# cloneofsimo/paint-with-words-sd

Measured on NVIDIA H100. Metric: unet_steps_per_sec_512sq_cfg, higher is better.
Workload: dtype f16

## Files before the change

paint_with_words_sd_b200/csrc/pww_abi.cu:

```cuda
#include <stdio.h>
#include <string.h>

#include "pww_common.cuh"
#include "xattn_tc.cuh"
#include "xattn_fused2.cuh"
#include "attn_tc.cuh"
#include "unet_ops.cuh"
#include "sampler_step.cuh"
#include "control_inject.cuh"
#include "control_combine.cuh"
#include <stdlib.h>
#include <algorithm>
#include <type_traits>

namespace {

thread_local char g_last_cuda_error[640] = "";

int cuda_fail(cudaError_t e);

bool aligned16(const void* p) { return (reinterpret_cast<uintptr_t>(p) & 15u) == 0; }

bool supported_head_dim(int D) { return D == 40 || D == 64 || D == 80 || D == 160; }

int check_common(const void* q, const void* k, int B, int H, int N, int T, int D, int64_t q_bs, int64_t q_rs,
                 int64_t k_bs, int64_t k_rs) {
  if (!q || !k || B <= 0 || H <= 0 || N <= 0 || T <= 0 || D <= 0) return PWW_ERR_BAD_ARG;
  if (!aligned16(q) || !aligned16(k)) return PWW_ERR_BAD_ARG;
  if ((q_bs | q_rs | k_bs | k_rs) & 7) return PWW_ERR_BAD_ARG;
  if (q_rs < (int64_t)H * D || k_rs < (int64_t)H * D) return PWW_ERR_BAD_ARG;
  if (!supported_head_dim(D) || !pww::core::supported_keys(T)) return PWW_ERR_UNSUPPORTED;
  return PWW_OK;
}

template <int D_, int KC_>
struct Shape {
  static constexpr int D = D_, KC = KC_;
};
template <int D, typename F>
cudaError_t with_chunks(int T, F&& f) {
  switch (pww::core::chunks_of(T)) {
    case 1: return f(Shape<D, 1>{});
    case 2: return f(Shape<D, 2>{});
    case 3: return f(Shape<D, 3>{});
  }
  return cudaErrorInvalidValue;
}
template <typename F>
cudaError_t with_shape(int D, int T, F&& f) {
  switch (D) {
    case 40: return with_chunks<40>(T, f);
    case 64: return with_chunks<64>(T, f);
    case 80: return with_chunks<80>(T, f);
    case 160: return with_chunks<160>(T, f);
  }
  return cudaErrorInvalidValue;
}

template <int lo, int hi, typename F>
void with_int(int v, F&& f) {
  if constexpr (lo < hi)
    if (v != lo) return with_int<lo + 1, hi>(v, f);
  f(std::integral_constant<int, lo>{});
}

size_t align_up(size_t x, size_t a) { return (x + a - 1) / a * a; }

constexpr int kStatSlotsPerImage = 2048;

int cuda_fail(cudaError_t e) {
  snprintf(g_last_cuda_error, sizeof(g_last_cuda_error), "%s: %s ", cudaGetErrorName(e), cudaGetErrorString(e));
  return PWW_ERR_CUDA;
}

template <typename E>
pww::XattnParams<E> xattn_params(const void* q, const void* k, const void* v, void* out, int B, int H, int N, int T, int D,
                                 int64_t q_bs, int64_t q_rs, int64_t k_bs, int64_t k_rs, int64_t o_bs, int64_t o_rs) {
  pww::XattnParams<E> p;
  memset(&p, 0, sizeof(p));
  p.q = (const E*)q; p.k = (const E*)k; p.v = (const E*)v; p.out = (E*)out;
  p.B = B; p.H = H; p.N = N; p.T = T; p.D = D;
  p.q_bs = q_bs; p.q_rs = q_rs; p.k_bs = k_bs; p.k_rs = k_rs; p.o_bs = o_bs; p.o_rs = o_rs;
  return p;
}

template <typename E>
pww::XattnParams<E> images(const pww::XattnParams<E>& p, int b0, int n) {
  pww::XattnParams<E> c = p;
  c.B = n;
  c.q += (int64_t)b0 * p.q_bs;
  c.k += (int64_t)b0 * p.k_bs;
  if (c.v) c.v += (int64_t)b0 * p.k_bs;
  if (c.out) c.out += (int64_t)b0 * p.o_bs;
  if (c.wmap_index) c.wmap_index += b0;
  if (c.stat_kind) c.stat_kind += b0;
  if (c.stats) c.stats += b0;
  if (c.stats_out) c.stats_out += b0;
  if (c.g_sigma) c.g_sigma += (int64_t)b0 * p.g_stride;
  return c;
}

}

extern "C" {

int pww_version(void) { return 300; }

const char* pww_status_str(int status) {
  switch (status) {
    case PWW_OK: return "ok";
    case PWW_ERR_BAD_ARG: return "bad argument (null/misaligned pointer, non-positive size or stride not a multiple of 8)";
    case PWW_ERR_UNSUPPORTED: return "unsupported shape or dtype (head dim must be 40/64/80/160, T <= 80, 154 or 231)";
    case PWW_ERR_CUDA: return "CUDA error (see pww_last_cuda_error)";
    case PWW_ERR_WORKSPACE: return "workspace too small (see pww_xattn_workspace_bytes)";
    default: return "unknown status";
  }
}

const char* pww_last_cuda_error(void) { return g_last_cuda_error; }

int pww_device_supported(void) {
  int dev = 0, major = 0;
  cudaError_t e = cudaGetDevice(&dev);
  if (e != cudaSuccess) return cuda_fail(e);
  e = cudaDeviceGetAttribute(&major, cudaDevAttrComputeCapabilityMajor, dev);
  if (e != cudaSuccess) return cuda_fail(e);
  return major == 9 ? 1 : 0;
}

size_t pww_xattn_workspace_bytes(int B, int H, int N, int T, int D) {
  (void)T; (void)D;
  if (B <= 0 || H <= 0 || N <= 0) return 0;
  return align_up((size_t)B * sizeof(unsigned int), 256) +
         (size_t)B * kStatSlotsPerImage * sizeof(pww::StatPartial);
}

}

namespace {

template <typename E>
int xattn_stats(const void* q, const void* k, int B, int H, int N, int T, int D, int64_t q_batch_stride,
                int64_t q_row_stride, int64_t k_batch_stride, int64_t k_row_stride, int stat, const int32_t* kinds,
                bool per_image, const int32_t* wmap_index, float* stats, void* workspace, size_t workspace_bytes,
                void* stream) {
  int rc = check_common(q, k, B, H, N, T, D, q_batch_stride, q_row_stride, k_batch_stride, k_row_stride);
  if (rc) return rc;
  if (!stats || !workspace) return PWW_ERR_BAD_ARG;
  if (per_image ? !kinds : (stat != PWW_STAT_MAX && stat != PWW_STAT_STD)) return PWW_ERR_BAD_ARG;
  if (workspace_bytes < pww_xattn_workspace_bytes(B, H, N, T, D)) return PWW_ERR_WORKSPACE;
  if (pww::num_sms() > kStatSlotsPerImage) return PWW_ERR_WORKSPACE;
  pww::XattnParams<E> p = xattn_params<E>(q, k, nullptr, nullptr, B, H, N, T, D, q_batch_stride, q_row_stride,
                                          k_batch_stride, k_row_stride, 0, 0);
  p.wmap_index = wmap_index; p.stat = stat; p.stat_kind = per_image ? kinds : nullptr; p.stats_out = stats;
  p.counters = (unsigned int*)workspace;
  p.partials = (pww::StatPartial*)((char*)workspace + align_up((size_t)B * sizeof(unsigned int), 256));
  for (int b0 = 0; b0 < B; b0 += pww::tc::kMaxBatch) {
    const pww::XattnParams<E> c = images(p, b0, std::min(B - b0, pww::tc::kMaxBatch));
    const cudaError_t e =
        with_shape(D, T, [&](auto k) { return pww::tc::launch_stats<k.D, k.KC>(c, (cudaStream_t)stream); });
    if (e != cudaSuccess) return cuda_fail(e);
  }
  return PWW_OK;
}

template <typename E>
int xattn_fwd(const void* q, const void* k, const void* v, void* out, int B, int H, int N, int T, int D,
              int64_t q_batch_stride, int64_t q_row_stride, int64_t k_batch_stride, int64_t k_row_stride,
              int64_t o_batch_stride, int64_t o_row_stride, const float* wmap, int64_t wmap_batch_stride,
              const int32_t* wmap_index, const float* stats, const float* g_sigma, int64_t g_stride, float scale,
              void* stream) {
  int rc = check_common(q, k, B, H, N, T, D, q_batch_stride, q_row_stride, k_batch_stride, k_row_stride);
  if (rc) return rc;
  if (!v || !out || !aligned16(v) || !aligned16(out)) return PWW_ERR_BAD_ARG;
  if ((o_batch_stride | o_row_stride) & 7 || o_row_stride < (int64_t)H * D) return PWW_ERR_BAD_ARG;
  if (wmap && (!stats || !g_sigma)) return PWW_ERR_BAD_ARG;
  pww::XattnParams<E> p = xattn_params<E>(q, k, v, out, B, H, N, T, D, q_batch_stride, q_row_stride, k_batch_stride,
                                          k_row_stride, o_batch_stride, o_row_stride);
  p.wmap = wmap; p.wmap_bs = wmap_batch_stride; p.wmap_index = wmap ? wmap_index : nullptr;
  p.stats = stats; p.g_sigma = g_sigma; p.g_stride = g_stride; p.scale = scale;
  for (int b0 = 0; b0 < B; b0 += pww::tc::kMaxBatch) {
    pww::XattnParams<E> c = images(p, b0, std::min(B - b0, pww::tc::kMaxBatch));
    if (wmap && !wmap_index) c.wmap += (int64_t)b0 * wmap_batch_stride;
    const cudaError_t e =
        with_shape(D, T, [&](auto k) { return pww::tc::launch_fwd<k.D, k.KC>(c, (cudaStream_t)stream); });
    if (e != cudaSuccess) return cuda_fail(e);
  }
  return PWW_OK;
}

template <typename E>
int xattn_fused(const void* q, const void* k, const void* v, void* out, int B, int H, int N, int T, int D,
                int64_t q_batch_stride, int64_t q_row_stride, int64_t k_batch_stride, int64_t k_row_stride,
                int64_t o_batch_stride, int64_t o_row_stride, const void* mpack, int64_t mpack_batch_stride, int Bw,
                const int8_t* cidx, const int32_t* wmap_index, int stat, const int32_t* kinds, bool per_image,
                const float* g_sigma, float scale, float* stats, void* workspace, size_t workspace_bytes,
                void* stream) {
  int rc = check_common(q, k, B, H, N, T, D, q_batch_stride, q_row_stride, k_batch_stride, k_row_stride);
  if (rc) return rc;
  if (!v || !out || !aligned16(v) || !aligned16(out)) return PWW_ERR_BAD_ARG;
  if ((o_batch_stride | o_row_stride) & 7 || o_row_stride < (int64_t)H * D || o_batch_stride <= 0) return PWW_ERR_BAD_ARG;
  if (mpack) {
    if (!cidx || !g_sigma || !workspace || Bw <= 0 || !aligned16(mpack)) return PWW_ERR_BAD_ARG;
    if ((mpack_batch_stride & 7) || mpack_batch_stride < (int64_t)N * pww::fx::kMW) return PWW_ERR_BAD_ARG;
    if (per_image ? !kinds : (stat != PWW_STAT_MAX && stat != PWW_STAT_STD)) return PWW_ERR_BAD_ARG;
    if (workspace_bytes < pww_xattn_fused_workspace_bytes()) return PWW_ERR_WORKSPACE;
  }
  pww::XattnParams<E> p = xattn_params<E>(q, k, v, out, B, H, N, T, D, q_batch_stride, q_row_stride, k_batch_stride,
                                          k_row_stride, o_batch_stride, o_row_stride);
  p.g_sigma = g_sigma; p.g_stride = per_image ? 1 : 0; p.scale = scale; p.stat = stat;
  p.stat_kind = per_image ? kinds : nullptr; p.stats_out = stats;
  p.wmap_index = mpack ? wmap_index : nullptr;
  p.counters = (unsigned int*)workspace;
  p.partials = workspace ? (pww::StatPartial*)((char*)workspace + 512) : nullptr;
  int chunk = pww::fx::kMaxBatch;
  const int tiles = pww::ceil_div(N, pww::core::kBM);
  const int hg = pww::ceil_div(H, D == 40 ? pww::fx::Cfg2<40>::G : (D == 64 ? pww::fx::Cfg2<64>::G : 1));
  while (chunk > 1) {
    const int cb = B < chunk ? B : chunk;
    if (pww::fx::fused2_fits(cb, hg, tiles, pww::fx::fused_grid(cb * hg * tiles))) break;
    chunk >>= 1;
  }
  for (int b0 = 0; b0 < B; b0 += chunk) {
    pww::XattnParams<E> c = images(p, b0, std::min(B - b0, chunk));
    const void* mp = mpack;
    const int8_t* ci = cidx;
    if (mpack && !wmap_index) {
      mp = (const __half*)mpack + (int64_t)b0 * mpack_batch_stride;
      ci = cidx + (int64_t)b0 * pww::core::kTP * pww::core::chunks_of(T);
    }
    c.wmap = (const float*)mp;
    const cudaError_t e = with_shape(D, T, [&](auto k) {
      return pww::fx::launch_fused2<k.D, k.KC>(c, mp, mpack_batch_stride, ci, (cudaStream_t)stream);
    });
    if (e == cudaErrorInvalidConfiguration) return PWW_ERR_UNSUPPORTED;
    if (e != cudaSuccess) return cuda_fail(e);
  }
  return PWW_OK;
}

template <typename E>
int groupnorm_nhwc(const void* x, const void* add, int64_t add_batch_stride, const void* gamma, const void* beta, void* y,
                   int B, int HW, int C, int G, float eps, int silu, void* workspace, size_t workspace_bytes,
                   void* stream) {
  if (!x || !gamma || !beta || !y || !workspace || B <= 0 || HW <= 0 || C <= 0 || G <= 0) return PWW_ERR_BAD_ARG;
  if (!aligned16(x) || !aligned16(y) || !aligned16(gamma) || !aligned16(beta) || (add && !aligned16(add)))
    return PWW_ERR_BAD_ARG;
  if ((C & 7) || (C % G) || G > 64 || (C >> 3) > 1024) return PWW_ERR_UNSUPPORTED;
  if (add && ((add_batch_stride & 7) || add_batch_stride < C)) return PWW_ERR_BAD_ARG;
  if (workspace_bytes < pww_groupnorm_workspace_bytes(B, HW, G)) return PWW_ERR_WORKSPACE;
  pww::uops::GnParams<E> p;
  p.x = (const E*)x; p.add = (const E*)add; p.add_bs = add_batch_stride; p.gamma = (const E*)gamma; p.beta = (const E*)beta;
  p.y = (E*)y;
  char* w = (char*)workspace;
  p.counters = (unsigned int*)w;
  w += align_up((size_t)B * sizeof(unsigned int), 256);
  p.stats = (float*)w;
  w += align_up((size_t)B * G * 2 * sizeof(float), 256);
  p.partial = (float*)w;
  p.B = B; p.HW = HW; p.C = C; p.G = G; p.eps = eps; p.silu = silu;
  p.chunks = pww::uops::gn_chunks(HW);
  p.rows_per_chunk = (HW + p.chunks - 1) / p.chunks;
  cudaStream_t s = (cudaStream_t)stream;
  const int nvec = C >> 3;
  const int rpp = nvec >= 256 ? 1 : 256 / nvec;
  const size_t smem1 = (size_t)rpp * C * 2 * sizeof(float);
  if (smem1 > 48 * 1024) return PWW_ERR_UNSUPPORTED;
  pww::uops::gn_stats_kernel<E><<<dim3(p.chunks, B), nvec * rpp, smem1, s>>>(p);
  int rows_per_block = (int)(((long long)HW * B + 2 * pww::num_sms() - 1) / (2 * pww::num_sms()));
  if (rows_per_block < rpp) rows_per_block = rpp;
  if (rows_per_block > 32) rows_per_block = 32;
  pww::uops::gn_apply_kernel<E><<<dim3((HW + rows_per_block - 1) / rows_per_block, B), nvec * rpp, 0, s>>>(p, rows_per_block);
  cudaError_t e = cudaGetLastError();
  return e == cudaSuccess ? PWW_OK : cuda_fail(e);
}

template <typename E>
int geglu(const void* in, void* out, int64_t M, int I, void* stream) {
  if (!in || !out || M <= 0 || I <= 0 || !aligned16(in) || !aligned16(out)) return PWW_ERR_BAD_ARG;
  if (I & 7) return PWW_ERR_UNSUPPORTED;
  const long long total = (long long)M * (I >> 3);
  long long blocks = (total + 255) / 256;
  const long long cap = (long long)pww::num_sms() * 16;
  if (blocks > cap) blocks = cap;
  pww::uops::geglu_kernel<E><<<(int)blocks, 256, 0, (cudaStream_t)stream>>>((const E*)in, (E*)out, M, I);
  cudaError_t e = cudaGetLastError();
  return e == cudaSuccess ? PWW_OK : cuda_fail(e);
}

template <typename E>
int add_layernorm(const void* x, const void* res, const void* gamma, const void* beta, void* sum_out, void* y, int64_t M,
                  int C, float eps, void* stream) {
  if (!x || !gamma || !beta || !y || M <= 0 || C <= 0) return PWW_ERR_BAD_ARG;
  if (!aligned16(x) || !aligned16(y) || !aligned16(gamma) || !aligned16(beta) || (res && !aligned16(res)) ||
      (sum_out && !aligned16(sum_out)))
    return PWW_ERR_BAD_ARG;
  if ((C & 7) || C > 2048) return PWW_ERR_UNSUPPORTED;
  const int warps = 8;
  const unsigned grid = (unsigned)((M + warps - 1) / warps);
  with_int<1, 8>(((C >> 3) + 31) / 32, [&](auto vpl) {
    pww::uops::add_layernorm_kernel<E, vpl><<<grid, warps * 32, 0, (cudaStream_t)stream>>>(
        (const E*)x, (const E*)res, (const E*)gamma, (const E*)beta, (E*)sum_out, (E*)y, M, C, eps);
  });
  cudaError_t e = cudaGetLastError();
  return e == cudaSuccess ? PWW_OK : cuda_fail(e);
}

template <typename E>
int attn_fwd(const void* q, const void* k, const void* v, void* out, int B, int H, int N, int D, int64_t qkv_batch_stride,
             int64_t qkv_row_stride, int64_t o_batch_stride, int64_t o_row_stride, float scale, void* stream) {
  if (!q || !k || !v || !out || B <= 0 || H <= 0 || N <= 0 || D <= 0) return PWW_ERR_BAD_ARG;
  if (!aligned16(q) || !aligned16(k) || !aligned16(v) || !aligned16(out)) return PWW_ERR_BAD_ARG;
  if ((qkv_batch_stride | qkv_row_stride | o_batch_stride | o_row_stride) & 7) return PWW_ERR_BAD_ARG;
  if (qkv_row_stride < (int64_t)H * D || o_row_stride < (int64_t)H * D) return PWW_ERR_BAD_ARG;
  if (!supported_head_dim(D)) return PWW_ERR_UNSUPPORTED;
  const cudaError_t e = with_shape(D, 1, [&](auto sh) {
    return pww::fa::launch<sh.D, E>(q, k, v, out, B, H, N, qkv_batch_stride, qkv_row_stride, o_batch_stride,
                                    o_row_stride, scale, (cudaStream_t)stream);
  });
  return e == cudaSuccess ? PWW_OK : cuda_fail(e);
}

template <typename E>
int control_inject(int n, void* const* dst, const void* const* res, const int64_t* elems_per_image, int rows,
                   const float* scales, void* stream) {
  if (n < 1 || n > pww::ctl::kMaxLevels || rows < 1 || !dst || !res || !elems_per_image) return PWW_ERR_BAD_ARG;
  pww::ctl::InjectArgs a;
  a.off[0] = 0;
  for (int k = 0; k < n; ++k) {
    const int64_t e = elems_per_image[k];
    if (e <= 0 || (e % pww::ctl::kVec) != 0) return PWW_ERR_BAD_ARG;
    if (!dst[k] || !res[k] || !aligned16(dst[k]) || !aligned16(res[k])) return PWW_ERR_BAD_ARG;
    a.dst[k] = dst[k];
    a.res[k] = res[k];
    a.vec_per_image[k] = e / pww::ctl::kVec;
    a.off[k + 1] = a.off[k] + (int64_t)rows * a.vec_per_image[k];
  }
  for (int k = n; k < pww::ctl::kMaxLevels; ++k) {
    a.dst[k] = nullptr;
    a.res[k] = nullptr;
    a.vec_per_image[k] = 0;
    a.off[k + 1] = a.off[n];
  }
  a.scales = scales;
  a.n = n;
  a.rows = rows;
  const cudaError_t e = pww::ctl::launch_inject<E>(a, (int64_t)pww::num_sms() * 8, (cudaStream_t)stream);
  return e == cudaSuccess ? PWW_OK : cuda_fail(e);
}

template <typename E>
int control_combine(int units, int n, void* const* out, const void* const* res, const int64_t* elems_per_image,
                    int rows, const float* scales, void* stream) {
  if (units < 1 || units > pww::ctl::kMaxUnits || n < 1 || n > pww::ctl::kMaxLevels || rows < 1 || !out || !res ||
      !elems_per_image || !scales)
    return PWW_ERR_BAD_ARG;
  pww::ctl::CombineArgs a = {};
  for (int k = 0; k < n; ++k) {
    const int64_t e = elems_per_image[k];
    if (e <= 0 || (e % pww::ctl::kVec) != 0) return PWW_ERR_BAD_ARG;
    if (!out[k] || !aligned16(out[k])) return PWW_ERR_BAD_ARG;
    a.out[k] = out[k];
    a.vec_per_image[k] = e / pww::ctl::kVec;
    a.off[k + 1] = a.off[k] + (int64_t)rows * a.vec_per_image[k];
  }
  for (int i = 0; i < units * n; ++i) {
    if (!res[i] || !aligned16(res[i])) return PWW_ERR_BAD_ARG;
    a.res[i] = res[i];
  }
  for (int k = n; k < pww::ctl::kMaxLevels; ++k) a.off[k + 1] = a.off[n];
  a.scales = scales;
  a.units = units;
  a.n = n;
  a.rows = rows;
  const cudaError_t e = pww::ctl::launch_combine<E>(a, (int64_t)pww::num_sms() * 8, (cudaStream_t)stream);
  return e == cudaSuccess ? PWW_OK : cuda_fail(e);
}

}

extern "C" {

int pww_xattn_stats_f16(const void* q, const void* k, int B, int H, int N, int T, int D, int64_t q_batch_stride,
    int64_t q_row_stride, int64_t k_batch_stride, int64_t k_row_stride, int stat, const int32_t* wmap_index,
    float* stats, void* workspace, size_t workspace_bytes, void* stream) {
  return xattn_stats<__half>(
      q, k, B, H, N, T, D, q_batch_stride, q_row_stride, k_batch_stride, k_row_stride, stat, nullptr, false,
      wmap_index, stats, workspace, workspace_bytes, stream);
}
int pww_xattn_stats_bf16(const void* q, const void* k, int B, int H, int N, int T, int D, int64_t q_batch_stride,
    int64_t q_row_stride, int64_t k_batch_stride, int64_t k_row_stride, int stat, const int32_t* wmap_index,
    float* stats, void* workspace, size_t workspace_bytes, void* stream) {
  return xattn_stats<__nv_bfloat16>(
      q, k, B, H, N, T, D, q_batch_stride, q_row_stride, k_batch_stride, k_row_stride, stat, nullptr, false,
      wmap_index, stats, workspace, workspace_bytes, stream);
}

int pww_xattn_stats_multi_f16(const void* q, const void* k, int B, int H, int N, int T, int D, int64_t q_batch_stride,
    int64_t q_row_stride, int64_t k_batch_stride, int64_t k_row_stride, const int32_t* stat, const int32_t* wmap_index,
    float* stats, void* workspace, size_t workspace_bytes, void* stream) {
  return xattn_stats<__half>(
      q, k, B, H, N, T, D, q_batch_stride, q_row_stride, k_batch_stride, k_row_stride, PWW_STAT_MAX, stat, true,
      wmap_index, stats, workspace, workspace_bytes, stream);
}
int pww_xattn_stats_multi_bf16(const void* q, const void* k, int B, int H, int N, int T, int D, int64_t q_batch_stride,
    int64_t q_row_stride, int64_t k_batch_stride, int64_t k_row_stride, const int32_t* stat, const int32_t* wmap_index,
    float* stats, void* workspace, size_t workspace_bytes, void* stream) {
  return xattn_stats<__nv_bfloat16>(
      q, k, B, H, N, T, D, q_batch_stride, q_row_stride, k_batch_stride, k_row_stride, PWW_STAT_MAX, stat, true,
      wmap_index, stats, workspace, workspace_bytes, stream);
}

int pww_xattn_fwd_f16(const void* q, const void* k, const void* v, void* out, int B, int H, int N, int T, int D,
    int64_t q_batch_stride, int64_t q_row_stride, int64_t k_batch_stride, int64_t k_row_stride, int64_t o_batch_stride,
    int64_t o_row_stride, const float* wmap, int64_t wmap_batch_stride, const int32_t* wmap_index, const float* stats,
    const float* g_sigma, float scale, void* stream) {
  return xattn_fwd<__half>(q, k, v, out, B, H, N, T, D, q_batch_stride, q_row_stride, k_batch_stride, k_row_stride,
      o_batch_stride, o_row_stride, wmap, wmap_batch_stride, wmap_index, stats, g_sigma, 0, scale, stream);
}
int pww_xattn_fwd_bf16(const void* q, const void* k, const void* v, void* out, int B, int H, int N, int T, int D,
    int64_t q_batch_stride, int64_t q_row_stride, int64_t k_batch_stride, int64_t k_row_stride, int64_t o_batch_stride,
    int64_t o_row_stride, const float* wmap, int64_t wmap_batch_stride, const int32_t* wmap_index, const float* stats,
    const float* g_sigma, float scale, void* stream) {
  return xattn_fwd<__nv_bfloat16>(
      q, k, v, out, B, H, N, T, D, q_batch_stride, q_row_stride, k_batch_stride, k_row_stride,
      o_batch_stride, o_row_stride, wmap, wmap_batch_stride, wmap_index, stats, g_sigma, 0, scale, stream);
}

int pww_xattn_fwd_multi_f16(const void* q, const void* k, const void* v, void* out, int B, int H, int N, int T, int D,
    int64_t q_batch_stride, int64_t q_row_stride, int64_t k_batch_stride, int64_t k_row_stride, int64_t o_batch_stride,
    int64_t o_row_stride, const float* wmap, int64_t wmap_batch_stride, const int32_t* wmap_index, const float* stats,
    const float* g_sigma, float scale, void* stream) {
  return xattn_fwd<__half>(q, k, v, out, B, H, N, T, D, q_batch_stride, q_row_stride, k_batch_stride, k_row_stride,
      o_batch_stride, o_row_stride, wmap, wmap_batch_stride, wmap_index, stats, g_sigma, 1, scale, stream);
}
int pww_xattn_fwd_multi_bf16(const void* q, const void* k, const void* v, void* out, int B, int H, int N, int T, int D,
    int64_t q_batch_stride, int64_t q_row_stride, int64_t k_batch_stride, int64_t k_row_stride, int64_t o_batch_stride,
    int64_t o_row_stride, const float* wmap, int64_t wmap_batch_stride, const int32_t* wmap_index, const float* stats,
    const float* g_sigma, float scale, void* stream) {
  return xattn_fwd<__nv_bfloat16>(
      q, k, v, out, B, H, N, T, D, q_batch_stride, q_row_stride, k_batch_stride, k_row_stride,
      o_batch_stride, o_row_stride, wmap, wmap_batch_stride, wmap_index, stats, g_sigma, 1, scale, stream);
}

size_t pww_xattn_fused_workspace_bytes(void) { return pww::fx::fused_workspace_bytes(); }

int pww_xattn_fused_f16(const void* q, const void* k, const void* v, void* out, int B, int H, int N, int T, int D,
    int64_t q_batch_stride, int64_t q_row_stride, int64_t k_batch_stride, int64_t k_row_stride, int64_t o_batch_stride,
    int64_t o_row_stride, const void* mpack, int64_t mpack_batch_stride, int Bw, const int8_t* cidx,
    const int32_t* wmap_index, int stat, const float* g_sigma, float scale, float* stats, void* workspace,
    size_t workspace_bytes, void* stream) {
  return xattn_fused<__half>(q, k, v, out, B, H, N, T, D, q_batch_stride, q_row_stride, k_batch_stride, k_row_stride,
      o_batch_stride, o_row_stride, mpack, mpack_batch_stride, Bw, cidx, wmap_index, stat, nullptr, false,
      g_sigma, scale, stats, workspace, workspace_bytes, stream);
}
int pww_xattn_fused_bf16(const void* q, const void* k, const void* v, void* out, int B, int H, int N, int T, int D,
    int64_t q_batch_stride, int64_t q_row_stride, int64_t k_batch_stride, int64_t k_row_stride, int64_t o_batch_stride,
    int64_t o_row_stride, const void* mpack, int64_t mpack_batch_stride, int Bw, const int8_t* cidx,
    const int32_t* wmap_index, int stat, const float* g_sigma, float scale, float* stats, void* workspace,
    size_t workspace_bytes, void* stream) {
  return xattn_fused<__nv_bfloat16>(
      q, k, v, out, B, H, N, T, D, q_batch_stride, q_row_stride, k_batch_stride, k_row_stride,
      o_batch_stride, o_row_stride, mpack, mpack_batch_stride, Bw, cidx, wmap_index, stat, nullptr, false,
      g_sigma, scale, stats, workspace, workspace_bytes, stream);
}

int pww_xattn_fused_multi_f16(const void* q, const void* k, const void* v, void* out, int B, int H, int N, int T, int D,
    int64_t q_batch_stride, int64_t q_row_stride, int64_t k_batch_stride, int64_t k_row_stride, int64_t o_batch_stride,
    int64_t o_row_stride, const void* mpack, int64_t mpack_batch_stride, int Bw, const int8_t* cidx,
// ... 150 lines not shown
```

paint_with_words_sd_b200/csrc/xattn_core.cuh:

```cuda
#pragma once
#include "mma_sm90.cuh"
#include "pww_common.cuh"

namespace pww {
namespace core {

constexpr int kBM = 128;
constexpr int kTP = 80;
constexpr int kWarps = 8;
constexpr int kThreads = kWarps * 32;

template <int D>
struct Tile {
  static_assert(D == 40 || D == 64 || D == 80 || D == 160, "head dims of SD1.5 (40 / 80 / 160) and SD2.x (64)");
  static constexpr int DP = (D + 15) / 16 * 16;
  static constexpr int LD = DP + 8;
  static constexpr int KS = DP / 16;
  static constexpr int NT = D / 8;
  static constexpr uint32_t QBYTES = kBM * LD * 2;
  static constexpr uint32_t KBYTES = kTP * LD * 2;
};

template <int D, typename E>
__device__ __forceinline__ void load_rows(uint32_t dst, const E* src, int64_t rs, int nrows, int valid) {
  using C = Tile<D>;
  constexpr int CH = C::DP / 8, DCH = D / 8;
  for (int idx = threadIdx.x; idx < nrows * CH; idx += blockDim.x) {
    const int r = idx / CH, c = idx - r * CH;
    const bool ok = r < valid && c < DCH;
    ptx::cp_async16(dst + (uint32_t)(r * C::LD + c * 8) * 2u, ok ? (const void*)(src + (int64_t)r * rs + c * 8) : (const void*)src,
                    ok ? 16u : 0u);
  }
}

template <int D, typename E>
__device__ __forceinline__ void warp_qk(uint32_t qs, uint32_t ks, int lane, float (&s)[10][4]) {
  using C = Tile<D>;
#pragma unroll
  for (int j = 0; j < 10; ++j) s[j][0] = s[j][1] = s[j][2] = s[j][3] = 0.f;
#pragma unroll
  for (int kk = 0; kk < C::KS; ++kk) {
    uint32_t a[4];
    ptx::ldsm_x4(qs + (uint32_t)((lane & 15) * C::LD + kk * 16 + (lane >> 4) * 8) * 2u, a[0], a[1], a[2], a[3]);
#pragma unroll
    for (int jp = 0; jp < 5; ++jp) {
      const int t = 16 * jp + (lane & 7) + ((lane >> 4) << 3), d = kk * 16 + ((lane >> 3) & 1) * 8;
      uint32_t b0, b1, b2, b3;
      ptx::ldsm_x4(ks + (uint32_t)(t * C::LD + d) * 2u, b0, b1, b2, b3);
      ptx::mma16816<E>(s[2 * jp], a, b0, b1);
      ptx::mma16816<E>(s[2 * jp + 1], a, b2, b3);
    }
  }
}

__device__ __forceinline__ int tok(int j, int e, int lane) { return 8 * j + 2 * (lane & 3) + (e & 1); }

template <int D, typename E>
__device__ __forceinline__ void warp_store(const float (&o)[Tile<D>::NT][4], unsigned char* stage, int lane, E* out,
                                           int64_t o_rs, int row0, int N) {
  using C = Tile<D>;
  __syncwarp();
  const int g = lane >> 2, q = lane & 3;
#pragma unroll
  for (int j = 0; j < C::NT; ++j) {
    *reinterpret_cast<uint32_t*>(stage + (g * C::LD + 8 * j + 2 * q) * 2) = ptx::pack2<E>(o[j][0], o[j][1]);
    *reinterpret_cast<uint32_t*>(stage + ((g + 8) * C::LD + 8 * j + 2 * q) * 2) = ptx::pack2<E>(o[j][2], o[j][3]);
  }
  __syncwarp();
  for (int idx = lane; idx < 16 * C::NT; idx += 32) {
    const int r = idx / C::NT, c = idx - r * C::NT;
    if (row0 + r < N)
      *reinterpret_cast<uint4*>(out + (int64_t)(row0 + r) * o_rs + c * 8) =
          *reinterpret_cast<const uint4*>(stage + (r * C::LD + c * 8) * 2);
  }
  __syncwarp();
}

constexpr int kChunk = 77;
constexpr int kMaxChunks = 3;
__host__ __device__ __forceinline__ constexpr int chunks_of(int T) { return T <= kTP ? 1 : T / kChunk; }
__host__ __device__ __forceinline__ constexpr bool supported_keys(int T) {
  return T <= kTP || T == 2 * kChunk || T == kMaxChunks * kChunk;
}
template <int KC>
__host__ __device__ __forceinline__ constexpr int chunk_keys(int T) { return KC == 1 ? T : kChunk; }

template <int D, int KC, typename E>
__device__ __forceinline__ void load_operands(uint32_t st, const XattnParams<E>& p, int b, int h, int tile, bool with_v) {
  using C = Tile<D>;
  const int rows = p.N - tile * kBM;
  load_rows<D>(st, p.q + (int64_t)b * p.q_bs + (int64_t)tile * kBM * p.q_rs + h * D, p.q_rs, kBM, rows < kBM ? rows : kBM);
  const int kv = chunk_keys<KC>(p.T);
#pragma unroll 1
  for (int c = 0; c < KC; ++c) {
    const int64_t off = (int64_t)b * p.k_bs + (int64_t)c * kChunk * p.k_rs + h * D;
    load_rows<D>(st + C::QBYTES + c * C::KBYTES, p.k + off, p.k_rs, kTP, kv);
    if (with_v) load_rows<D>(st + C::QBYTES + (KC + c) * C::KBYTES, p.v + off, p.k_rs, kTP, kv);
  }
}

template <int D>
__device__ __forceinline__ void warp_online_begin(float (&o)[Tile<D>::NT][4], float& m0, float& m1, float& l0, float& l1) {
#pragma unroll
  for (int j = 0; j < Tile<D>::NT; ++j) o[j][0] = o[j][1] = o[j][2] = o[j][3] = 0.f;
  m0 = m1 = -INFINITY;
  l0 = l1 = 0.f;
}

template <int D, typename E, int NJ>
__device__ __forceinline__ void warp_online_chunk(float (&s)[NJ][4], int kv, float sl2, uint32_t vs, int lane,
                                                  float (&o)[Tile<D>::NT][4], float& m0, float& m1, float& l0, float& l1) {
  static_assert(NJ % 2 == 0, "P V takes two n-tiles of P per k-step");
  using C = Tile<D>;
  float t0 = -INFINITY, t1 = -INFINITY;
#pragma unroll
  for (int j = 0; j < NJ; ++j)
#pragma unroll
    for (int e = 0; e < 4; ++e) {
      if (tok(j, e, lane) >= kv) s[j][e] = -INFINITY;
      if (e < 2) t0 = fmaxf(t0, s[j][e]); else t1 = fmaxf(t1, s[j][e]);
    }
  t0 = fmaxf(t0, __shfl_xor_sync(0xffffffffu, t0, 1));
  t0 = fmaxf(t0, __shfl_xor_sync(0xffffffffu, t0, 2));
  t1 = fmaxf(t1, __shfl_xor_sync(0xffffffffu, t1, 1));
  t1 = fmaxf(t1, __shfl_xor_sync(0xffffffffu, t1, 2));
  const float mn0 = fmaxf(m0, t0), mn1 = fmaxf(m1, t1);
  const float a0 = ptx::ex2((m0 - mn0) * sl2), a1 = ptx::ex2((m1 - mn1) * sl2);
  m0 = mn0; m1 = mn1;
  const float n0 = -mn0 * sl2, n1 = -mn1 * sl2;
  uint32_t pa[NJ / 2][4];
  float r0 = 0.f, r1 = 0.f;
#pragma unroll
  for (int j = 0; j < NJ; ++j) {
    const uint32_t p01 = ptx::pack2<E>(ptx::ex2(fmaf(s[j][0], sl2, n0)), ptx::ex2(fmaf(s[j][1], sl2, n0)));
    const uint32_t p23 = ptx::pack2<E>(ptx::ex2(fmaf(s[j][2], sl2, n1)), ptx::ex2(fmaf(s[j][3], sl2, n1)));
    const float2 f01 = ptx::unpack2<E>(p01), f23 = ptx::unpack2<E>(p23);
    r0 += f01.x + f01.y;
    r1 += f23.x + f23.y;
    pa[j >> 1][(j & 1) * 2] = p01;
    pa[j >> 1][(j & 1) * 2 + 1] = p23;
  }
  l0 = l0 * a0 + r0;
  l1 = l1 * a1 + r1;
#pragma unroll
  for (int j = 0; j < C::NT; ++j) {
    o[j][0] *= a0; o[j][1] *= a0; o[j][2] *= a1; o[j][3] *= a1;
  }
#pragma unroll
  for (int kk = 0; kk < NJ / 2; ++kk) {
    const int t = 16 * kk + (lane & 7) + ((lane >> 3) & 1) * 8;
#pragma unroll
    for (int jp = 0; jp < C::NT / 2; ++jp) {
      uint32_t b0, b1, b2, b3;
      ptx::ldsm_x4_t(vs + (uint32_t)(t * C::LD + 16 * jp + (lane >> 4) * 8) * 2u, b0, b1, b2, b3);
      ptx::mma16816<E>(o[2 * jp], pa[kk], b0, b1);
      ptx::mma16816<E>(o[2 * jp + 1], pa[kk], b2, b3);
    }
    if constexpr (C::NT & 1) {
      uint32_t b0, b1;
      ptx::ldsm_x2_t(vs + (uint32_t)(t * C::LD + 8 * (C::NT - 1)) * 2u, b0, b1);
      ptx::mma16816<E>(o[C::NT - 1], pa[kk], b0, b1);
    }
  }
}

template <int D>
__device__ __forceinline__ void warp_online_end(float (&o)[Tile<D>::NT][4], float l0, float l1) {
  l0 += __shfl_xor_sync(0xffffffffu, l0, 1);
  l0 += __shfl_xor_sync(0xffffffffu, l0, 2);
  l1 += __shfl_xor_sync(0xffffffffu, l1, 1);
  l1 += __shfl_xor_sync(0xffffffffu, l1, 2);
  const float i0 = 1.f / l0, i1 = 1.f / l1;
#pragma unroll
  for (int j = 0; j < Tile<D>::NT; ++j) {
    o[j][0] *= i0; o[j][1] *= i0; o[j][2] *= i1; o[j][3] *= i1;
  }
}

template <typename E>
__device__ __forceinline__ void warp_stat(const float (&s)[10][4], int T, int rows_left, int lane, bool is_max, float& vmax,
                                          float& sum, float& sumsq) {
  const int g = lane >> 2;
#pragma unroll
  for (int j = 0; j < 10; ++j)
#pragma unroll
    for (int e = 0; e < 4; ++e) {
      const bool ok = tok(j, e, lane) < T && (g + (e >> 1) * 8) < rows_left;
      if (is_max) {
        if (ok) vmax = fmaxf(vmax, s[j][e]);
      } else if (ok) {
        const float h = round_to<E>(s[j][e]);
        sum += h;
        sumsq = fmaf(h, h, sumsq);
      }
    }
}

__device__ __forceinline__ void warp_reduce_stat(double& m, double& a, double& q) {
#pragma unroll
  for (int o = 16; o > 0; o >>= 1) {
    m = fmax(m, __shfl_xor_sync(0xffffffffu, m, o));
    a += __shfl_xor_sync(0xffffffffu, a, o);
    q += __shfl_xor_sync(0xffffffffu, q, o);
  }
}

template <typename E>
__device__ __forceinline__ float stat_value(const XattnParams<E>& p, bool is_max, double m, double a, double q) {
  const double cnt = (double)p.H * (double)p.N * (double)p.T;
  double r;
  if (is_max) {
    r = m;
  } else {
    const double var = (q - a * a / cnt) / (cnt - 1.0);
    r = sqrt(var > 0.0 ? var : 0.0);
  }
  return round_to<E>((float)r);
}

}
}
```

Baseline: 145.9.

## Add warp-specialized WGMMA flash attention for long self-attention sequences

Adds a Hopper self-attention kernel with producer warps that load K/V tiles into a multi-stage shared-memory ring tracked by mbarriers. Two consumer warpgroups issue asynchronous wgmma for QK and PV, overlapping one tile's softmax with the previous tile's PV product and alternating turns via named barriers. The softmax helper is split out so both kernels share it, and dispatch uses the new kernel for head dims 40/64/80 when N is at least 1024. This targets the mma.sync issue and load-latency limits of the old kernel, at the cost of complex synchronisation, register redistribution through setmaxnreg, and descriptor layout risk.

```diff
diff --git a/paint_with_words_sd_b200/csrc/attn_wgmma.cuh b/paint_with_words_sd_b200/csrc/attn_wgmma.cuh
--- /dev/null
+++ b/paint_with_words_sd_b200/csrc/attn_wgmma.cuh
@@ -0,0 +1,306 @@
+#pragma once
+#include "mma_sm90.cuh"
+#include "pww_common.cuh"
+#include "xattn_core.cuh"
+
+namespace pww {
+namespace wg {
+
+constexpr int kBM = 128;
+constexpr int kBN = 128;
+constexpr int kMaxStages = 8;
+constexpr int kConsumers = 256;
+constexpr int kProducers = 128;
+constexpr int kThreads = kConsumers + kProducers;
+constexpr int kProducerRegs = 40, kConsumerRegs = 232;
+static_assert(kProducers * kProducerRegs + kConsumers * kConsumerRegs <= 65536 / kThreads / 8 * 8 * kThreads,
+              "setmaxnreg moves registers between the warpgroups of the CTA's own allocation");
+
+__device__ __forceinline__ uint64_t smem_desc(uint32_t addr, uint32_t lbo, uint32_t sbo) {
+  return (uint64_t)((addr & 0x3FFFFu) >> 4) | ((uint64_t)(lbo >> 4) << 16) | ((uint64_t)(sbo >> 4) << 32);
+}
+
+template <int D>
+struct Cfg {
+  static_assert(D == 40 || D == 64 || D == 80, "head dims with an m64nDk16 P V shape");
+  static constexpr int DP = (D + 15) / 16 * 16;
+  static constexpr int KCH = DP / 8;
+  static constexpr int VCH = D / 8;
+  static constexpr int KS = DP / 16;
+  static constexpr uint32_t QBYTES = kBM * DP * 2;
+  static constexpr uint32_t KBYTES = kBN * DP * 2;
+  static constexpr uint32_t STAGE = KBYTES + kBN * D * 2;
+  static constexpr uint32_t OFF_KV = QBYTES;
+  static constexpr uint32_t OUTBYTES = kBM * core::Tile<D>::LD * 2;
+  static constexpr int ST_FIT = (int)((232448u - QBYTES - OUTBYTES - 2 * kMaxStages * 8) / STAGE);
+  static constexpr int ST = ST_FIT < kMaxStages ? ST_FIT : kMaxStages;
+  static constexpr uint32_t OFF_OUT = OFF_KV + ST * STAGE;
+  static constexpr uint32_t OFF_BAR = OFF_OUT + OUTBYTES;
+  static constexpr uint32_t SMEM = OFF_BAR + 2 * ST * 8;
+  static_assert(SMEM <= 232448, "shared memory budget");
+  static_assert(QBYTES % 128 == 0 && STAGE % 128 == 0, "core matrices stay 128-byte aligned");
+};
+
+template <typename E>
+struct Params {
+  const E* q;
+  const E* k;
+  const E* v;
+  E* out;
+  int B, H, N;
+  int64_t bs, rs;
+  int64_t o_bs, o_rs;
+  float scale;
+};
+
+__device__ __forceinline__ void mbar_init(uint32_t bar, unsigned count) {
+  asm volatile("mbarrier.init.shared::cta.b64 [%0], %1;" ::"r"(bar), "r"(count) : "memory");
+}
+__device__ __forceinline__ void mbar_wait(uint32_t bar, unsigned parity) {
+  asm volatile(
+      "{\n.reg .pred done;\nWAIT_%=:\n"
+      "mbarrier.try_wait.parity.shared::cta.b64 done, [%0], %1;\n"
+      "@!done bra WAIT_%=;\n}\n" ::"r"(bar), "r"(parity) : "memory");
+}
+__device__ __forceinline__ void mbar_arrive(uint32_t bar) {
+  asm volatile("mbarrier.arrive.shared::cta.b64 _, [%0];" ::"r"(bar) : "memory");
+}
+__device__ __forceinline__ void cp_async_mbar_arrive(uint32_t bar) {
+  asm volatile("cp.async.mbarrier.arrive.noinc.shared::cta.b64 [%0];" ::"r"(bar) : "memory");
+}
+__device__ __forceinline__ void cp_async16_ca(uint32_t dst, const void* src, uint32_t src_bytes) {
+  asm volatile("cp.async.ca.shared.global [%0], [%1], 16, %2;" ::"r"(dst), "l"(src), "r"(src_bytes) : "memory");
+}
+__device__ __forceinline__ void fence_proxy_async() { asm volatile("fence.proxy.async.shared::cta;" ::: "memory"); }
+
+__device__ __forceinline__ void wgmma_fence() { asm volatile("wgmma.fence.sync.aligned;" ::: "memory"); }
+__device__ __forceinline__ void wgmma_commit() { asm volatile("wgmma.commit_group.sync.aligned;" ::: "memory"); }
+__device__ __forceinline__ void bar_sync(int id) { asm volatile("bar.sync %0, %1;" ::"r"(id), "n"(kConsumers) : "memory"); }
+__device__ __forceinline__ void bar_arrive(int id) { asm volatile("bar.arrive %0, %1;" ::"r"(id), "n"(kConsumers) : "memory"); }
+template <int N>
+__device__ __forceinline__ void wgmma_wait() { asm volatile("wgmma.wait_group.sync.aligned %0;" ::"n"(N) : "memory"); }
+template <int R>
+__device__ __forceinline__ void fence_regs(float (&d)[R][4]) {
+#pragma unroll
+  for (int i = 0; i < R; ++i)
+#pragma unroll
+    for (int e = 0; e < 4; ++e) asm volatile("" : "+f"(d[i][e])::"memory");
+}
+
+#define PWW_WGMMA_QK(T) \
+  asm volatile( \
+      "{\n.reg .pred p;\nsetp.ne.b32 p, %66, 0;\n" \
+      "wgmma.mma_async.sync.aligned.m64n128k16.f32." T "." T " {" \
+      "%0, %1, %2, %3, %4, %5, %6, %7, %8, %9, %10, %11, %12, %13, %14, %15, " \
+      "%16, %17, %18, %19, %20, %21, %22, %23, %24, %25, %26, %27, %28, %29, %30, %31, " \
+      "%32, %33, %34, %35, %36, %37, %38, %39, %40, %41, %42, %43, %44, %45, %46, %47, " \
+      "%48, %49, %50, %51, %52, %53, %54, %55, %56, %57, %58, %59, %60, %61, %62, %63}, %64, %65, p, 1, 1, 0, 0;\n}\n" \
+      : "+f"(d[0][0]), "+f"(d[0][1]), "+f"(d[0][2]), "+f"(d[0][3]), "+f"(d[1][0]), "+f"(d[1][1]), "+f"(d[1][2]), "+f"(d[1][3]), \
+        "+f"(d[2][0]), "+f"(d[2][1]), "+f"(d[2][2]), "+f"(d[2][3]), "+f"(d[3][0]), "+f"(d[3][1]), "+f"(d[3][2]), "+f"(d[3][3]), \
+        "+f"(d[4][0]), "+f"(d[4][1]), "+f"(d[4][2]), "+f"(d[4][3]), "+f"(d[5][0]), "+f"(d[5][1]), "+f"(d[5][2]), "+f"(d[5][3]), \
+        "+f"(d[6][0]), "+f"(d[6][1]), "+f"(d[6][2]), "+f"(d[6][3]), "+f"(d[7][0]), "+f"(d[7][1]), "+f"(d[7][2]), "+f"(d[7][3]), \
+        "+f"(d[8][0]), "+f"(d[8][1]), "+f"(d[8][2]), "+f"(d[8][3]), "+f"(d[9][0]), "+f"(d[9][1]), "+f"(d[9][2]), "+f"(d[9][3]), \
+        "+f"(d[10][0]), "+f"(d[10][1]), "+f"(d[10][2]), "+f"(d[10][3]), "+f"(d[11][0]), "+f"(d[11][1]), "+f"(d[11][2]), "+f"(d[11][3]), \
+        "+f"(d[12][0]), "+f"(d[12][1]), "+f"(d[12][2]), "+f"(d[12][3]), "+f"(d[13][0]), "+f"(d[13][1]), "+f"(d[13][2]), "+f"(d[13][3]), \
+        "+f"(d[14][0]), "+f"(d[14][1]), "+f"(d[14][2]), "+f"(d[14][3]), "+f"(d[15][0]), "+f"(d[15][1]), "+f"(d[15][2]), "+f"(d[15][3]) \
+      : "l"(da), "l"(db), "r"(accumulate))
+#define PWW_WGMMA_PV40(T) \
+  asm volatile( \
+      "{\n.reg .pred p;\nsetp.ne.b32 p, %25, 0;\n" \
+      "wgmma.mma_async.sync.aligned.m64n40k16.f32." T "." T " {" \
+      "%0, %1, %2, %3, %4, %5, %6, %7, %8, %9, %10, %11, %12, %13, %14, %15, " \
+      "%16, %17, %18, %19}, {%20, %21, %22, %23}, %24, p, 1, 1, 1;\n}\n" \
+      : "+f"(d[0][0]), "+f"(d[0][1]), "+f"(d[0][2]), "+f"(d[0][3]), "+f"(d[1][0]), "+f"(d[1][1]), "+f"(d[1][2]), "+f"(d[1][3]), \
+        "+f"(d[2][0]), "+f"(d[2][1]), "+f"(d[2][2]), "+f"(d[2][3]), "+f"(d[3][0]), "+f"(d[3][1]), "+f"(d[3][2]), "+f"(d[3][3]), \
+        "+f"(d[4][0]), "+f"(d[4][1]), "+f"(d[4][2]), "+f"(d[4][3]) \
+      : "r"(a[0]), "r"(a[1]), "r"(a[2]), "r"(a[3]), "l"(db), "r"(1))
+#define PWW_WGMMA_PV64(T) \
+  asm volatile( \
+      "{\n.reg .pred p;\nsetp.ne.b32 p, %37, 0;\n" \
+      "wgmma.mma_async.sync.aligned.m64n64k16.f32." T "." T " {" \
+      "%0, %1, %2, %3, %4, %5, %6, %7, %8, %9, %10, %11, %12, %13, %14, %15, " \
+      "%16, %17, %18, %19, %20, %21, %22, %23, %24, %25, %26, %27, %28, %29, %30, %31}, {%32, %33, %34, %35}, %36, p, 1, 1, 1;\n}\n" \
+      : "+f"(d[0][0]), "+f"(d[0][1]), "+f"(d[0][2]), "+f"(d[0][3]), "+f"(d[1][0]), "+f"(d[1][1]), "+f"(d[1][2]), "+f"(d[1][3]), \
+        "+f"(d[2][0]), "+f"(d[2][1]), "+f"(d[2][2]), "+f"(d[2][3]), "+f"(d[3][0]), "+f"(d[3][1]), "+f"(d[3][2]), "+f"(d[3][3]), \
+        "+f"(d[4][0]), "+f"(d[4][1]), "+f"(d[4][2]), "+f"(d[4][3]), "+f"(d[5][0]), "+f"(d[5][1]), "+f"(d[5][2]), "+f"(d[5][3]), \
+        "+f"(d[6][0]), "+f"(d[6][1]), "+f"(d[6][2]), "+f"(d[6][3]), "+f"(d[7][0]), "+f"(d[7][1]), "+f"(d[7][2]), "+f"(d[7][3]) \
+      : "r"(a[0]), "r"(a[1]), "r"(a[2]), "r"(a[3]), "l"(db), "r"(1))
+#define PWW_WGMMA_PV80(T) \
+  asm volatile( \
+      "{\n.reg .pred p;\nsetp.ne.b32 p, %45, 0;\n" \
+      "wgmma.mma_async.sync.aligned.m64n80k16.f32." T "." T " {" \
+      "%0, %1, %2, %3, %4, %5, %6, %7, %8, %9, %10, %11, %12, %13, %14, %15, " \
+      "%16, %17, %18, %19, %20, %21, %22, %23, %24, %25, %26, %27, %28, %29, %30, %31, " \
+      "%32, %33, %34, %35, %36, %37, %38, %39}, {%40, %41, %42, %43}, %44, p, 1, 1, 1;\n}\n" \
+      : "+f"(d[0][0]), "+f"(d[0][1]), "+f"(d[0][2]), "+f"(d[0][3]), "+f"(d[1][0]), "+f"(d[1][1]), "+f"(d[1][2]), "+f"(d[1][3]), \
+        "+f"(d[2][0]), "+f"(d[2][1]), "+f"(d[2][2]), "+f"(d[2][3]), "+f"(d[3][0]), "+f"(d[3][1]), "+f"(d[3][2]), "+f"(d[3][3]), \
+        "+f"(d[4][0]), "+f"(d[4][1]), "+f"(d[4][2]), "+f"(d[4][3]), "+f"(d[5][0]), "+f"(d[5][1]), "+f"(d[5][2]), "+f"(d[5][3]), \
+        "+f"(d[6][0]), "+f"(d[6][1]), "+f"(d[6][2]), "+f"(d[6][3]), "+f"(d[7][0]), "+f"(d[7][1]), "+f"(d[7][2]), "+f"(d[7][3]), \
+        "+f"(d[8][0]), "+f"(d[8][1]), "+f"(d[8][2]), "+f"(d[8][3]), "+f"(d[9][0]), "+f"(d[9][1]), "+f"(d[9][2]), "+f"(d[9][3]) \
+      : "r"(a[0]), "r"(a[1]), "r"(a[2]), "r"(a[3]), "l"(db), "r"(1))
+
+template <typename E>
+__device__ __forceinline__ void mma_qk(float (&d)[16][4], uint64_t da, uint64_t db, int accumulate) {
+  if constexpr (std::is_same_v<E, __half>) PWW_WGMMA_QK("f16");
+  else PWW_WGMMA_QK("bf16");
+}
+template <int D, typename E>
+__device__ __forceinline__ void mma_pv(float (&d)[D / 8][4], const uint32_t (&a)[4], uint64_t db) {
+  constexpr bool f16 = std::is_same_v<E, __half>;
+  if constexpr (D == 40) { if constexpr (f16) PWW_WGMMA_PV40("f16"); else PWW_WGMMA_PV40("bf16"); }
+  if constexpr (D == 64) { if constexpr (f16) PWW_WGMMA_PV64("f16"); else PWW_WGMMA_PV64("bf16"); }
+  if constexpr (D == 80) { if constexpr (f16) PWW_WGMMA_PV80("f16"); else PWW_WGMMA_PV80("bf16"); }
+}
+
+template <int D, int CH, typename E>
+__device__ __forceinline__ void load_tile(uint32_t dst, const E* src, int64_t rs, int valid, int t) {
+#pragma unroll 1
+  for (int i = t; i < 128 * CH; i += kProducers) {
+    const int r = i / CH, c = i - r * CH;
+    const bool ok = r < valid && c < D / 8;
+    cp_async16_ca(dst + (uint32_t)(((r >> 3) * CH + c) * 128 + (r & 7) * 16),
+                  ok ? (const void*)(src + (int64_t)r * rs + c * 8) : (const void*)src, ok ? 16u : 0u);
+  }
+}
+
+template <int D, typename E>
+__global__ void __launch_bounds__(kThreads, 1) attn_fwd_kernel(const Params<E> p) {
+  using CF = Cfg<D>;
+  extern __shared__ __align__(128) unsigned char smem[];
+  const uint32_t smem0 = ptx::smem_u32(smem);
+  const uint32_t full = smem0 + CF::OFF_BAR, empty = full + 8 * CF::ST;
+  const int warp = threadIdx.x >> 5, lane = threadIdx.x & 31;
+  const int qtiles = (p.N + kBM - 1) / kBM;
+  const int bh = blockIdx.x / qtiles, qt = blockIdx.x - bh * qtiles;
+  const int b = bh / p.H, h = bh - b * p.H;
+  const int row_base = qt * kBM;
+  const int ntiles = (p.N + kBN - 1) / kBN;
+  if (threadIdx.x == 0) {
+    for (int s = 0; s < CF::ST; ++s) {
+      mbar_init(full + 8 * s, kProducers);
+      mbar_init(empty + 8 * s, kConsumers / 32);
+    }
+    asm volatile("fence.mbarrier_init.release.cluster;" ::: "memory");
+  }
+  __syncthreads();
+
+  if (threadIdx.x >= kConsumers) {
+    asm volatile("setmaxnreg.dec.sync.aligned.u32 %0;" ::"n"(kProducerRegs));
+    const int t = threadIdx.x - kConsumers;
+    const int64_t off = (int64_t)b * p.bs + h * D;
+#pragma unroll 1
+    for (int j = 0; j < ntiles; ++j) {
+      const int s = j % CF::ST;
+      if (j >= CF::ST) mbar_wait(empty + 8 * s, (j / CF::ST - 1) & 1);
+      if (j == 0) load_tile<D, CF::KCH>(smem0, p.q + off + (int64_t)row_base * p.rs, p.rs, p.N - row_base, t);
+      const uint32_t st = smem0 + CF::OFF_KV + s * CF::STAGE;
+      const int64_t row = (int64_t)j * kBN * p.rs;
+      load_tile<D, CF::KCH>(st, p.k + off + row, p.rs, p.N - j * kBN, t);
+      load_tile<D, CF::VCH>(st + CF::KBYTES, p.v + off + row, p.rs, p.N - j * kBN, t);
+      cp_async_mbar_arrive(full + 8 * s);
+    }
+    ptx::cp_async_wait<0>();
+    return;
+  }
+  asm volatile("setmaxnreg.inc.sync.aligned.u32 %0;" ::"n"(kConsumerRegs));
+
+  const int wgi = warp >> 2;
+  const float sl2 = p.scale * 1.4426950408889634f;
+  const uint64_t dq = smem_desc(smem0 + wgi * 64 * CF::DP * 2, 128, CF::KCH * 128);
+  auto dk = [&](int j) { return smem_desc(smem0 + CF::OFF_KV + (j % CF::ST) * CF::STAGE, 128, CF::KCH * 128); };
+  auto dv = [&](int j) {
+    return smem_desc(smem0 + CF::OFF_KV + (j % CF::ST) * CF::STAGE + CF::KBYTES, CF::VCH * 128, 128);
+  };
+  float s[16][4], o[D / 8][4], m0, m1, l0, l1;
+  core::warp_online_begin<D>(o, m0, m1, l0, l1);
+  uint32_t pa0[8][4], pa1[8][4];
+  auto turn_begin = [&]() { bar_sync(1 + wgi); };
+  auto turn_end = [&]() { bar_arrive(2 - wgi); };
+  if (wgi == 1) bar_arrive(1);
+  auto wait_full = [&](int j) {
+    mbar_wait(full + 8 * (j % CF::ST), (j / CF::ST) & 1);
+    fence_proxy_async();
+  };
+  auto issue_qk = [&](int j) {
+    const uint64_t k0 = dk(j);
+#pragma unroll
+    for (int kk = 0; kk < CF::KS; ++kk) mma_qk<E>(s, dq + 16 * kk, k0 + 16 * kk, kk);
+    wgmma_commit();
+  };
+  auto issue_pv = [&](int j, const uint32_t (&pa)[8][4]) {
+    const uint64_t v0 = dv(j);
+#pragma unroll
+    for (int kk = 0; kk < 8; ++kk) mma_pv<D, E>(o, pa[kk], v0 + 16 * CF::VCH * kk);
+    wgmma_commit();
+  };
+  auto softmax = [&](int j, uint32_t (&pa)[8][4], float& a0, float& a1) {
+    const int kv = p.N - j * kBN;
+    if (kv < kBN) core::warp_online_softmax<E>(s, kv, sl2, lane, m0, m1, l0, l1, pa, a0, a1);
+    else core::warp_online_softmax<E>(s, kBN, sl2, lane, m0, m1, l0, l1, pa, a0, a1);
+  };
+  auto step = [&](int j, const uint32_t (&pp)[8][4], uint32_t (&pn)[8][4]) {
+    wait_full(j);
+    wgmma_fence();
+    turn_begin();
+    issue_qk(j);
+    issue_pv(j - 1, pp);
+    turn_end();
+    wgmma_wait<1>();
+    fence_regs(s);
+    float a0, a1;
+    softmax(j, pn, a0, a1);
+    wgmma_wait<0>();
+    fence_regs(o);
+    if (lane == 0) mbar_arrive(empty + 8 * ((j - 1) % CF::ST));
+#pragma unroll
+    for (int i = 0; i < D / 8; ++i) {
+      o[i][0] *= a0; o[i][1] *= a0; o[i][2] *= a1; o[i][3] *= a1;
+    }
+  };
+
+  wait_full(0);
+  wgmma_fence();
+  turn_begin();
+  issue_qk(0);
+  turn_end();
+  wgmma_wait<0>();
+  fence_regs(s);
+  {
+    float a0, a1;
+    softmax(0, pa0, a0, a1);
+  }
+#pragma unroll 1
+  for (int j = 1; j < ntiles; j += 2) {
+    step(j, pa0, pa1);
+    if (j + 1 < ntiles) step(j + 1, pa1, pa0);
+  }
+  wgmma_fence();
+  turn_begin();
+  if ((ntiles - 1) & 1) issue_pv(ntiles - 1, pa1);
+  else issue_pv(ntiles - 1, pa0);
+  turn_end();
+  wgmma_wait<0>();
+  fence_regs(o);
+  if (wgi == 0) bar_sync(1);
+  core::warp_online_end<D>(o, l0, l1);
+  core::warp_store<D>(o, smem + CF::OFF_OUT + warp * 16 * core::Tile<D>::LD * 2, lane,
+                      p.out + (int64_t)b * p.o_bs + h * D, p.o_rs, row_base + warp * 16, p.N);
+}
+
+template <int D, typename E>
+cudaError_t launch(const void* q, const void* k, const void* v, void* out, int B, int H, int N, int64_t bs, int64_t rs,
+                   int64_t o_bs, int64_t o_rs, float scale, cudaStream_t s) {
+  using CF = Cfg<D>;
+  Params<E> p;
+  p.q = (const E*)q; p.k = (const E*)k; p.v = (const E*)v; p.out = (E*)out;
+  p.B = B; p.H = H; p.N = N; p.bs = bs; p.rs = rs; p.o_bs = o_bs; p.o_rs = o_rs; p.scale = scale;
+  const cudaError_t e = allow_dynamic_smem<attn_fwd_kernel<D, E>>(CF::SMEM);
+  if (e != cudaSuccess) return e;
+  const long long grid = (long long)B * H * ((N + kBM - 1) / kBM);
+  if (grid > 0x7fffffffLL) return cudaErrorInvalidConfiguration;
+  attn_fwd_kernel<D, E><<<(unsigned)grid, kThreads, CF::SMEM, s>>>(p);
+  return cudaGetLastError();
+}
+
+}
+}
diff --git a/paint_with_words_sd_b200/csrc/pww_abi.cu b/paint_with_words_sd_b200/csrc/pww_abi.cu
--- a/paint_with_words_sd_b200/csrc/pww_abi.cu
+++ b/paint_with_words_sd_b200/csrc/pww_abi.cu
@@ -5,6 +5,7 @@
 #include "xattn_tc.cuh"
 #include "xattn_fused2.cuh"
 #include "attn_tc.cuh"
+#include "attn_wgmma.cuh"
 #include "unet_ops.cuh"
 #include "sampler_step.cuh"
 #include "control_inject.cuh"
@@ -306,6 +307,8 @@
   return e == cudaSuccess ? PWW_OK : cuda_fail(e);
 }
 
+constexpr int kWgmmaMinKeys = 1024;
+
 template <typename E>
 int attn_fwd(const void* q, const void* k, const void* v, void* out, int B, int H, int N, int D, int64_t qkv_batch_stride,
              int64_t qkv_row_stride, int64_t o_batch_stride, int64_t o_row_stride, float scale, void* stream) {
@@ -315,6 +318,10 @@
   if (qkv_row_stride < (int64_t)H * D || o_row_stride < (int64_t)H * D) return PWW_ERR_BAD_ARG;
   if (!supported_head_dim(D)) return PWW_ERR_UNSUPPORTED;
   const cudaError_t e = with_shape(D, 1, [&](auto sh) {
+    if constexpr (sh.D != 160)
+      if (N >= kWgmmaMinKeys)
+        return pww::wg::launch<sh.D, E>(q, k, v, out, B, H, N, qkv_batch_stride, qkv_row_stride, o_batch_stride,
+                                        o_row_stride, scale, (cudaStream_t)stream);
     return pww::fa::launch<sh.D, E>(q, k, v, out, B, H, N, qkv_batch_stride, qkv_row_stride, o_batch_stride,
                                     o_row_stride, scale, (cudaStream_t)stream);
   });
diff --git a/paint_with_words_sd_b200/csrc/xattn_core.cuh b/paint_with_words_sd_b200/csrc/xattn_core.cuh
--- a/paint_with_words_sd_b200/csrc/xattn_core.cuh
+++ b/paint_with_words_sd_b200/csrc/xattn_core.cuh
@@ -107,11 +107,11 @@
   l0 = l1 = 0.f;
 }
 
-template <int D, typename E, int NJ>
-__device__ __forceinline__ void warp_online_chunk(float (&s)[NJ][4], int kv, float sl2, uint32_t vs, int lane,
-                                                  float (&o)[Tile<D>::NT][4], float& m0, float& m1, float& l0, float& l1) {
+template <typename E, int NJ>
+__device__ __forceinline__ void warp_online_softmax(float (&s)[NJ][4], int kv, float sl2, int lane, float& m0, float& m1,
+                                                    float& l0, float& l1, uint32_t (&pa)[NJ / 2][4], float& a0,
+                                                    float& a1) {
   static_assert(NJ % 2 == 0, "P V takes two n-tiles of P per k-step");
-  using C = Tile<D>;
   float t0 = -INFINITY, t1 = -INFINITY;
 #pragma unroll
   for (int j = 0; j < NJ; ++j)
@@ -125,10 +125,10 @@
   t1 = fmaxf(t1, __shfl_xor_sync(0xffffffffu, t1, 1));
   t1 = fmaxf(t1, __shfl_xor_sync(0xffffffffu, t1, 2));
   const float mn0 = fmaxf(m0, t0), mn1 = fmaxf(m1, t1);
-  const float a0 = ptx::ex2((m0 - mn0) * sl2), a1 = ptx::ex2((m1 - mn1) * sl2);
+  a0 = ptx::ex2((m0 - mn0) * sl2);
+  a1 = ptx::ex2((m1 - mn1) * sl2);
   m0 = mn0; m1 = mn1;
   const float n0 = -mn0 * sl2, n1 = -mn1 * sl2;
-  uint32_t pa[NJ / 2][4];
   float r0 = 0.f, r1 = 0.f;
 #pragma unroll
   for (int j = 0; j < NJ; ++j) {
@@ -142,6 +142,15 @@
   }
   l0 = l0 * a0 + r0;
   l1 = l1 * a1 + r1;
+}
+
+template <int D, typename E, int NJ>
+__device__ __forceinline__ void warp_online_chunk(float (&s)[NJ][4], int kv, float sl2, uint32_t vs, int lane,
+                                                  float (&o)[Tile<D>::NT][4], float& m0, float& m1, float& l0, float& l1) {
+  using C = Tile<D>;
+  uint32_t pa[NJ / 2][4];
+  float a0, a1;
+  warp_online_softmax<E>(s, kv, sl2, lane, m0, m1, l0, l1, pa, a0, a1);
 #pragma unroll
   for (int j = 0; j < C::NT; ++j) {
     o[j][0] *= a0; o[j][1] *= a0; o[j][2] *= a1; o[j][3] *= a1;
```

New measurement: 145.9 (median of 6 runs). No clear change (-0.0%).
